# GinZhu/RDST

Measured on AMD Instinct MI355X. Metric: SR patches/sec fwd+bwd, RDST-E1 x4 64->256, higher is better.
Workload: dtype bf16; 1 GPU; RDST-E1 x4 (RDST_E1_OASIS_example_SRx4.ini), 1x64x64 LR patches -> 256x256, step = fwd + L1 + bwd + flat-bucket grad all-reduce + Adam; global_batch=32, per_gpu_batch=32, parallelism=dp1, hip_graph=True, grad_bucket_bytes=17859844

## Files before the change

rdst_amd/csrc/mlp3_mfma.hip:

```cpp
#include "linear.h"
#include "lds_dma.h"
#include "mfma.h"

#ifndef M3_ABL
#define M3_ABL 0
#endif

namespace {

constexpr int M3_TT = 128;


struct M3Args {
  const bf16* X; int64_t ldx; int x_bytes;
  const bf16* W1p; const float* sb1;
  const bf16* W2p; const float* sb2;
  bf16* Y; int64_t ldy;
  float* stats;
  int M, ntiles;
  unsigned long long* stamps;
};

#ifndef M3_NW90
#define M3_NW90 12
#endif
constexpr int m3_nw(int C) { return ((2 * C + 31) / 32) % 3 == 0 ? M3_NW90 : 8; }

template <int C>
struct M3Cfg {
  static constexpr int HID = 2 * C;
  static constexpr int KS1 = (C + 15) / 16, NT1 = (HID + 31) / 32;
  static constexpr int KS2 = (HID + 15) / 16, NT2 = (C + 31) / 32;
  static constexpr int XS = lds_kstep_stride(C), XSLOTS = XS / 16, XD = (2 * C + 15) / 16;
  static constexpr int TP = (M3_TT * XSLOTS + 63) / 64, TILEB = TP * 1024;
  static constexpr int HS = lds_kstep_stride(HID), HTILEB = M3_TT * HS;
  static constexpr int NW = m3_nw(C), NTHR = 64 * NW;
  static constexpr int NJ1 = (NT1 * 4 + NW - 1) / NW, P1 = NT1 / ce_gcd(NW, NT1), ND1 = NJ1 < P1 ? NJ1 : P1;
  static constexpr int NJ2 = (NT2 * 4 + NW - 1) / NW, P2 = NT2 / ce_gcd(NW, NT2), ND2 = NJ2 < P2 ? NJ2 : P2;
  static constexpr int NBUF = 2;
  static constexpr int CNT = (TP + NW - 1) / NW;
  static constexpr int H_OFF = NBUF * TILEB;
  static constexpr int STAT_OFF = H_OFF + HTILEB;
  static constexpr int SB1_OFF = STAT_OFF + NBUF * M3_TT * 2 * 4;
  static constexpr int SB1_B = (2 * NT1 * 32 * 4 + 1023) / 1024 * 1024;
  static constexpr int SB2_OFF = SB1_OFF + SB1_B;
  static constexpr int SB2_B = (2 * NT2 * 32 * 4 + 1023) / 1024 * 1024;
  static constexpr int TAB_OFF = SB2_OFF + SB2_B;
  static constexpr int SMEM = TAB_OFF + RDST_GELU_TAB4_BYTES;
  static constexpr int WGCU = SMEM <= 80 * 1024 ? 2 : 1;
  static_assert(SMEM <= 160 * 1024, "LDS");
  static_assert(TP >= NW, "every wave owns at least one piece of a tile");
  static_assert(CNT + 1 + 2 * ((NT2 * 4) / NW) < 64, "vmcnt is a 6-bit counter");
};

template <int C>
__global__ void __launch_bounds__(64 * m3_nw(C), M3Cfg<C>::WGCU == 2 ? (2 * m3_nw(C) + 3) / 4 : (m3_nw(C) + 3) / 4) mlp3_fwd_kernel(const M3Args p) {
  using CF = M3Cfg<C>;
  constexpr int KS1 = CF::KS1, KS2 = CF::KS2, NT1 = CF::NT1, NT2 = CF::NT2, XS = CF::XS, HS = CF::HS, NBUF = CF::NBUF, NW = CF::NW;
  constexpr int ND1 = CF::ND1, ND2 = CF::ND2, NJ1 = CF::NJ1, NJ2 = CF::NJ2, CNT = CF::CNT;
  extern __shared__ __attribute__((aligned(16))) char smem[];
  const int tid = threadIdx.x, lane = tid & 63, r = lane & 31, h = lane >> 5;
  const int wave = __builtin_amdgcn_readfirstlane(tid >> 6);
  float* statL = reinterpret_cast<float*>(smem + CF::STAT_OFF);
  const float* sb1L = reinterpret_cast<const float*>(smem + CF::SB1_OFF);
  const float* sb2L = reinterpret_cast<const float*>(smem + CF::SB2_OFF);
  char* hL = smem + CF::H_OFF;
  gelu_tab4_fill(smem + CF::TAB_OFF, tid, CF::NTHR);
  const char* gtab = smem + CF::TAB_OFF;

  const u32x4s_t rsx = dma_rsrc(p.X, (uint32_t)p.x_bytes), rs1 = dma_rsrc(p.sb1, 2 * NT1 * 32 * 4), rs2 = dma_rsrc(p.sb2, 2 * NT2 * 32 * 4);
  const uint32_t lds0 = lds_base(smem);
  const int grid = gridDim.x;
  RDST_PHASES_BEGIN(RDST_DBGV(p.stamps));
  u32x4v_t w1[ND1][KS1], w2[ND2][KS2];
#pragma unroll
  for (int jd = 0; jd < ND1; ++jd) {
    const int nt = (wave + NW * jd) % NT1;
#pragma unroll
    for (int ks = 0; ks < KS1; ++ks) {
      const char* src = reinterpret_cast<const char*>(p.W1p) + (((int64_t)nt * KS1 + ks) * 64 + lane) * 16;
      frag_load(w1[jd][ks], src);
    }
  }
#pragma unroll
  for (int jd = 0; jd < ND2; ++jd) {
    const int nt = (wave + NW * jd) % NT2;
#pragma unroll
    for (int ks = 0; ks < KS2; ++ks) {
      const char* src = reinterpret_cast<const char*>(p.W2p) + (((int64_t)nt * KS2 + ks) * 64 + lane) * 16;
      frag_load(w2[jd][ks], src);
    }
  }
  {
    constexpr int N1P = CF::SB1_B / 1024, N2P = CF::SB2_B / 1024;
    const int p1 = wave % N1P, p2 = wave % N2P;
    lds_dma16(rs1, __builtin_amdgcn_readfirstlane(lds0 + (uint32_t)(CF::SB1_OFF + p1 * 1024)), p1 * 1024 + lane * 16);
    lds_dma16(rs2, __builtin_amdgcn_readfirstlane(lds0 + (uint32_t)(CF::SB2_OFF + p2 * 1024)), p2 * 1024 + lane * 16);
  }
  auto issue_tile = [&](int tile, int b) {
#pragma unroll
    for (int i = 0; i < CNT; ++i) {
      int q = wave + NW * i;
      q = q < CF::TP ? q : q - NW;
      const int sidx = q * 64 + lane;
      const int tok = sidx / CF::XSLOTS, sl = sidx - tok * CF::XSLOTS;
      const int grow = tile * M3_TT + tok;
      const bool ok = tile < p.ntiles && tok < M3_TT && sl < CF::XD && grow < p.M;
      lds_dma16(rsx, __builtin_amdgcn_readfirstlane(lds0 + (uint32_t)(b * CF::TILEB + q * 1024)),
          ok ? grow * ((int)p.ldx * 2) + sl * 16 : p.x_bytes);
    }
  };
  static_assert(NBUF == 2, "the ring below is written for two buffers");
  issue_tile(blockIdx.x, 0);
  issue_tile(blockIdx.x + grid, 1);
  constexpr int NST = 1 + 2 * ((NT2 * 4) / NW);
  int kk = 0;
  for (int tile = blockIdx.x; tile < p.ntiles; tile += grid, ++kk) {
    const int b = kk & 1;
    if (kk == 0) wait_vmcnt<CNT>();
    else wait_vmcnt<CNT + NST>();
#pragma unroll
    for (int jd = 0; jd < ND1; ++jd)
#pragma unroll
      for (int ks = 0; ks < KS1; ++ks) frag_pin(w1[jd][ks]);
#pragma unroll
    for (int jd = 0; jd < ND2; ++jd)
#pragma unroll
      for (int ks = 0; ks < KS2; ++ks) frag_pin(w2[jd][ks]);
    __syncthreads();
    RDST_PHASE(RDST_DBGV(p.stamps), 0);
    const char* tb = smem + b * CF::TILEB;
    float* st = statL + b * M3_TT * 2;
    for (int tok = tid >> 2; tok < M3_TT; tok += CF::NTHR / 4) {
      const int part = tid & 3;
      constexpr int NSL = (CF::XD + 3) / 4;
      float xv[NSL][8];
      float sum = 0.f;
#pragma unroll
      for (int i = 0; i < NSL; ++i) {
        const int sl = part + 4 * i;
        const Pack16 q = *reinterpret_cast<const Pack16*>(tb + tok * XS + (sl < CF::XD ? sl : 0) * 16);
        Mma<bf16>::unpack(q, xv[i]);
#pragma unroll
        for (int e = 0; e < 8; ++e) {
          const bool valid = sl < CF::XD && sl * 8 + e < C;
          xv[i][e] = valid ? xv[i][e] : 0.f;
          sum += xv[i][e];
        }
      }
      sum += __shfl_xor(sum, 1, 64);
      sum += __shfl_xor(sum, 2, 64);
      const float mean = sum * (1.0f / C);
      float sq = 0.f;
#pragma unroll
      for (int i = 0; i < NSL; ++i) {
        const int sl = part + 4 * i;
#pragma unroll
        for (int e = 0; e < 8; ++e) {
          const bool valid = sl < CF::XD && sl * 8 + e < C;
          const float d = xv[i][e] - mean;
          sq = valid ? fmaf(d, d, sq) : sq;
        }
      }
      sq += __shfl_xor(sq, 1, 64);
      sq += __shfl_xor(sq, 2, 64);
      const float rstd = rsqrtf(sq * (1.0f / C) + 1e-5f);
      if (part == 0) {
        st[tok * 2] = mean;
        st[tok * 2 + 1] = rstd;
        const int grow = tile * M3_TT + tok;
        if (grow < p.M) *reinterpret_cast<float2*>(p.stats + (int64_t)grow * 2) = make_float2(mean, rstd);
      }
    }
    __syncthreads();
    RDST_PHASE(RDST_DBGV(p.stamps), 1);
#pragma unroll
    for (int jd = 0; jd < ND1; ++jd)
#pragma unroll 1
      for (int j = jd; j < NJ1; j += ND1) {
        const int item = wave + NW * j;
        if (item >= NT1 * 4) break;
        const int nt = item % NT1, tt = item / NT1;
        const int tok = tt * 32 + r;
        f32x16 acc;
#pragma unroll
        for (int v = 0; v < 16; ++v) acc[v] = 0.f;
        const char* brow = tb + tok * XS + h * 16;
#pragma unroll
        for (int ks = 0; ks < KS1; ++ks) {
          Pack16 bq = *reinterpret_cast<const Pack16*>(brow + ks * 32);
          if (C % 16 != 0 && ks == KS1 - 1) {
            constexpr int c0 = C % 16 < 8 ? C % 16 : 8, c1 = C % 16 > 8 ? C % 16 - 8 : 0;
#pragma unroll
            for (int d = 0; d < 4; ++d) bq.w[d] = (2 * d < (h ? c1 : c0)) ? bq.w[d] : 0u;
          }
          if (!(M3_ABL & 2)) acc = __builtin_amdgcn_mfma_f32_32x32x16_bf16(__builtin_bit_cast(bf16x8_t, w1[jd][ks]), __builtin_bit_cast(bf16x8_t, bq), acc, 0, 0, 0);
          else acc[ks & 15] += __uint_as_float(bq.w[0]);
        }
        const float2 mr = *reinterpret_cast<const float2*>(st + tok * 2);
        const float rstd = mr.y, nrm = -mr.y * mr.x;
        char* hrow = hL + tok * HS;
        float u[16], fr[16];
        uint32_t en[16];
#pragma unroll
        for (int g4 = 0; g4 < 4; ++g4) {
          const int n0 = nt * 32 + 8 * g4 + 4 * h;
          const float4 S4 = *reinterpret_cast<const float4*>(sb1L + n0);
          const float4 B4 = *reinterpret_cast<const float4*>(sb1L + NT1 * 32 + n0);
          u[4 * g4] = fmaf(rstd, acc[4 * g4], fmaf(nrm, S4.x, B4.x));
          u[4 * g4 + 1] = fmaf(rstd, acc[4 * g4 + 1], fmaf(nrm, S4.y, B4.y));
          u[4 * g4 + 2] = fmaf(rstd, acc[4 * g4 + 2], fmaf(nrm, S4.z, B4.z));
          u[4 * g4 + 3] = fmaf(rstd, acc[4 * g4 + 3], fmaf(nrm, S4.w, B4.w));
        }
#pragma unroll
        for (int v = 0; v < 16; ++v) {
          uint32_t off;
          if (M3_ABL & 1) { fr[v] = 0.f; en[v] = 0x3c003c00u; continue; }
          fr[v] = gelu_tab4_index(u[v], off);
          en[v] = *reinterpret_cast<const uint32_t*>(gtab + off);
        }
        __builtin_amdgcn_sched_barrier(0);
#pragma unroll
        for (int g4 = 0; g4 < 4; ++g4) {
          const int n0 = nt * 32 + 8 * g4 + 4 * h;
          const float h0 = u[4 * g4] * gelu_tab_lerp(fr[4 * g4], en[4 * g4]), h1 = u[4 * g4 + 1] * gelu_tab_lerp(fr[4 * g4 + 1], en[4 * g4 + 1]);
          const float h2 = u[4 * g4 + 2] * gelu_tab_lerp(fr[4 * g4 + 2], en[4 * g4 + 2]), h3 = u[4 * g4 + 3] * gelu_tab_lerp(fr[4 * g4 + 3], en[4 * g4 + 3]);
          u32x2_a4 uu;
          uu.x = pack_bf16x2(h0, h1); uu.y = pack_bf16x2(h2, h3);
          if (n0 * 2 + 8 <= HS) *reinterpret_cast<u32x2_a4*>(hrow + n0 * 2) = uu;
        }
      }
    RDST_PHASE(RDST_DBGV(p.stamps), 2);
    __syncthreads();
    RDST_PHASE(RDST_DBGV(p.stamps), 3);
#pragma unroll
    for (int jd = 0; jd < ND2; ++jd)
#pragma unroll 1
      for (int j = jd; j < NJ2; j += ND2) {
        const int item = wave + NW * j;
        if (item >= NT2 * 4) break;
        const int nt = item % NT2, tt = item / NT2;
        const int tok = tt * 32 + r;
        const int grow = tile * M3_TT + tok;
        f32x16 acc;
#pragma unroll
        for (int v = 0; v < 16; ++v) acc[v] = 0.f;
        const char* brow = hL + tok * HS + h * 16;
#pragma unroll
        for (int ks = 0; ks < KS2; ++ks) {
          const Pack16 bq = *reinterpret_cast<const Pack16*>(brow + ks * 32);
          if (!(M3_ABL & 4)) acc = __builtin_amdgcn_mfma_f32_32x32x16_bf16(__builtin_bit_cast(bf16x8_t, w2[jd][ks]), __builtin_bit_cast(bf16x8_t, bq), acc, 0, 0, 0);
          else acc[ks & 15] += __uint_as_float(bq.w[0]);
        }
#pragma unroll
        for (int g4 = 0; g4 < 4; ++g4) {
          const int n0 = nt * 32 + 8 * g4 + 4 * h;
          const float4 B4 = *reinterpret_cast<const float4*>(sb2L + NT2 * 32 + n0);
          uint32_t rx = 0u, ry = 0u;
          if (n0 < C) {
            const u32x2_a4 rr = *reinterpret_cast<const u32x2_a4*>(tb + tok * XS + n0 * 2);
            rx = rr.x; ry = rr.y;
          }
          acc[4 * g4] += B4.x + bf16lo(rx); acc[4 * g4 + 1] += B4.y + bf16hi(rx);
          acc[4 * g4 + 2] += B4.z + bf16lo(ry); acc[4 * g4 + 3] += B4.w + bf16hi(ry);
        }
        if (grow < p.M && !(M3_ABL & 8)) {
#pragma unroll
          for (int gp = 0; gp < 2; ++gp) {
            float c8[8];
#pragma unroll
            for (int e = 0; e < 4; ++e) {
              const auto sw = __builtin_amdgcn_permlane32_swap(__float_as_uint(acc[8 * gp + e]), __float_as_uint(acc[8 * gp + 4 + e]),
                                                               false, false);
              c8[e] = __uint_as_float(sw[0]);
              c8[4 + e] = __uint_as_float(sw[1]);
            }
            const int cb = nt * 32 + 8 * (2 * gp + h);
            const int nv = C - cb;
            if (nv <= 0) continue;
            bf16* yp = p.Y + (grow * (int)p.ldy + cb);
            if (nv >= 8) {
              u32x4_a4 u;
              u.x = pack_bf16x2(c8[0], c8[1]); u.y = pack_bf16x2(c8[2], c8[3]);
              u.z = pack_bf16x2(c8[4], c8[5]); u.w = pack_bf16x2(c8[6], c8[7]);
              *reinterpret_cast<u32x4_a4*>(yp) = u;
            } else {
#pragma unroll
              for (int d = 0; d < 3; ++d)
                if (2 * d + 2 <= nv) *reinterpret_cast<uint32_t*>(yp + 2 * d) = pack_bf16x2(c8[2 * d], c8[2 * d + 1]);
            }
          }
        }
      }
    RDST_PHASE(RDST_DBGV(p.stamps), 4);
    __syncthreads();
    issue_tile(tile + 2 * grid, b);
    RDST_PHASE(RDST_DBGV(p.stamps), 5);
  }
  RDST_PHASES_STORE(RDST_DBGV(p.stamps) && tid == 0, p.stamps, blockIdx.x);
}

template <int C>
int launch_m3(M3Args& p, hipStream_t st) {
  using CF = M3Cfg<C>;
  p.ntiles = (p.M + M3_TT - 1) / M3_TT;
  int grid = (p.ntiles + 1) / 2;
  if (grid > 256 * CF::WGCU) grid = 256 * CF::WGCU;
  if (grid < 1) grid = 1;
  auto kern = mlp3_fwd_kernel<C>;
  p.stamps = rdst_stamps_begin("RDST_M3_STAMPS", grid, 8, st);
  const int rc = rdst_launch(kern, dim3((unsigned)grid), dim3(CF::NTHR), CF::SMEM, st, "mlp3_fwd", p);
  rdst_stamps_end(p.stamps, grid, 8, RDST_STAMPS_SUMS, st, "mlp3_fwd: 0 wait+B0, 1 stats, 2 phase 1, 3 wait+B2, 4 phase 2, 5 B3+issue");
  return rc;
}

}

size_t mlp3_pack_bytes(int C, int hid) { return lin3_pack_bytes(C, hid) + lin3_pack_bytes(hid, C); }

bool mlp3_fwd_shape(int C, int hid) { return hid == 2 * C && (C == 60 || C == 90 || C == 120); }

int mlp3_fwd_bf16(const bf16* X, int64_t ldx, const float* ln_w, const float* ln_b, const float* W1, const float* b1, const float* W2,
                  const float* b2, bf16* Y, int64_t ldy, float* stats, int64_t M, int C, int hid, void* wpack, bool prepacked,
                  hipStream_t st) {
  if (!wpack || ((uintptr_t)wpack & 15) || !mlp3_fwd_shape(C, hid) || M <= 0) return RDST_ENOTSUP;
  if (((uintptr_t)X & 3) || (ldx & 1) || ((uintptr_t)Y & 3) || (ldy & 1)) return RDST_ENOTSUP;
  const int64_t xb = ((M - 1) * ldx + C) * 2;
  if (xb >= (1ll << 31) || M * ldy * 2 >= (1ll << 31)) return RDST_ENOTSUP;
  char* base = reinterpret_cast<char*>(wpack);
  char* base2 = base + lin3_pack_bytes(C, hid);
  if (!prepacked) {
    if (int rc = lin3_pack_launch(W1, ln_w, ln_b, b1, base, hid, C, 1.0f, st)) return rc;
    if (int rc = lin3_pack_launch(W2, nullptr, nullptr, b2, base2, C, hid, 1.0f, st)) return rc;
  }
  const int nt1 = (hid + 31) / 32, ks1 = (C + 15) / 16, nt2 = (C + 31) / 32, ks2 = (hid + 15) / 16;
  M3Args p{};
  p.X = X; p.ldx = ldx; p.x_bytes = (int)xb;
  p.W1p = reinterpret_cast<const bf16*>(base); p.sb1 = reinterpret_cast<const float*>(base + (size_t)nt1 * ks1 * 1024);
  p.W2p = reinterpret_cast<const bf16*>(base2); p.sb2 = reinterpret_cast<const float*>(base2 + (size_t)nt2 * ks2 * 1024);
  p.Y = Y; p.ldy = ldy; p.stats = stats; p.M = (int)M;
  if (C == 60) return launch_m3<60>(p, st);
  if (C == 90) return launch_m3<90>(p, st);
  return launch_m3<120>(p, st);
}
```

rdst_amd/csrc/mlp_mfma.hip:

```cpp
#include "linear.h"
#include "mfma.h"
#include "reduce_batch.h"
#include "wattn_hd.h"
#include <stdlib.h>

#ifdef MLP_ABL
#define MLP_DBG(p) (MLP_ABL)
#else
#define MLP_DBG(p) RDST_DBGV((p).dbg)
#endif

namespace {
using namespace wahd;
using MM = Mma<bf16>;

struct MlpArgs {
  const bf16* X; int64_t ldx; const float* stats; const float* lnw; const float* lnb;
  const float* W1; const float* b1; const float* W2; const float* b2;
  const bf16* dY; int64_t lddy; bf16* dX; int64_t lddx;
  float* slab; int64_t slab_stride;
  int64_t M; int C; int hid; int64_t ntiles; int tiles_per_wg;
  unsigned long long* stamps;
  int dbg;
};

template <int NCT> struct MlpCfg {
  static constexpr int NJ = 2 * NCT, NT = 64 * NJ, CP = 32 * NCT, JP = 32 * NJ;
  static constexpr int KC = CP / 16, KJ = JP / 16, PK = CP / 8;
  static constexpr int LDW = NCT == 4 ? 336 : CP * 2 + 16, LDX = LDW, LDH = 64;
  static constexpr int OFF_W1 = 0, OFF_XH = OFF_W1 + JP * LDW, OFF_DY = OFF_XH + 32 * LDX, OFF_DH = OFF_DY + 32 * LDX,
                       OFF_B1 = OFF_DH + JP * LDH, OFF_SM = OFF_B1 + JP * 4, OFF_RED = OFF_SM + 32 * 4,
                       OFF_TAB = OFF_RED + NCT * 32 * 8, OFF_W2L = OFF_TAB + RDST_GELU_TAB_BYTES;
  static constexpr int W2L = NCT == 4 ? 3 : 0, SMEM = OFF_W2L + W2L * NJ * 1024;
};

__device__ __forceinline__ void gelu_pair(f32x2 x, f32x2& cdf, f32x2& ex) {
  const f32x2 z = x * 0.70710678118654752440f;
  f32x2 az;
  az.x = __builtin_fabsf(z.x); az.y = __builtin_fabsf(z.y);
  const f32x2 den = __builtin_elementwise_fma(az, (f32x2)(0.3275911f), (f32x2)(1.0f));
  f32x2 t;
  t.x = __builtin_amdgcn_rcpf(den.x); t.y = __builtin_amdgcn_rcpf(den.y);
  f32x2 pl = __builtin_elementwise_fma(t, (f32x2)(0.5f * 1.061405429f), (f32x2)(0.5f * -1.453152027f));
  pl = __builtin_elementwise_fma(pl, t, (f32x2)(0.5f * 1.421413741f));
  pl = __builtin_elementwise_fma(pl, t, (f32x2)(0.5f * -0.284496736f));
  pl = __builtin_elementwise_fma(pl, t, (f32x2)(0.5f * 0.254829592f));
  pl = pl * t;
  const f32x2 a2 = (z * -1.4426950408889634f) * z;
  ex.x = __builtin_amdgcn_exp2f(a2.x); ex.y = __builtin_amdgcn_exp2f(a2.y);
  const f32x2 qn = pl * ex, qp = (f32x2)(1.0f) - qn;
  cdf.x = x.x >= 0.f ? qp.x : qn.x;
  cdf.y = x.y >= 0.f ? qp.y : qn.y;
}

template <int NCT, bool SPLIT>
__global__ void __launch_bounds__(128 * NCT, 2) mlp_bwd_kernel(const MlpArgs p) {
  using CF = MlpCfg<NCT>;
  extern __shared__ __attribute__((aligned(16))) char smem[];
  constexpr int NT = CF::NT, JP = CF::JP, LDW = CF::LDW, LDX = CF::LDX, PK = CF::PK, NJ = CF::NJ;
  const int tid = threadIdx.x, lane = tid & 63, wave = __builtin_amdgcn_readfirstlane(tid >> 6), r = lane & 31, hh = lane >> 5;
  const int C = p.C, hid = p.hid;
  const int j = 32 * wave + r;
  float* b1s = reinterpret_cast<float*>(smem + CF::OFF_B1);
  float* sm = reinterpret_cast<float*>(smem + CF::OFF_SM);
  float* red = reinterpret_cast<float*>(smem + CF::OFF_RED);
  const lds_cp gtab = (lds_cp)(smem + CF::OFF_TAB);
  gelu_tab_fill(smem + CF::OFF_TAB, tid, NT);
  int nst = 0;
  auto stamp = [&]() {
    if (RDST_DBGV(p.stamps) && tid == 0 && nst < 14) p.stamps[(size_t)blockIdx.x * 16 + nst++] = __builtin_readcyclecounter();
  };
  stamp();

  Pack16 w2b[CF::KC - CF::W2L];
  const lds_cp w2l = (lds_cp)(smem + CF::OFF_W2L + (wave * 64 + lane) * 16);
  {
    float f[CF::KC][8];
#pragma unroll
    for (int t = 0; t < CF::KC; ++t)
#pragma unroll
      for (int e = 0; e < 8; ++e) {
        const int c = 16 * t + 8 * hh + e;
        f[t][e] = p.W2[(int64_t)(c < C ? c : C - 1) * hid + (j < hid ? j : hid - 1)];
      }
#pragma unroll
    for (int t = 0; t < CF::KC; ++t) {
#pragma unroll
      for (int e = 0; e < 8; ++e) f[t][e] = (16 * t + 8 * hh + e < C && j < hid) ? f[t][e] : 0.f;
      if (t < CF::KC - CF::W2L) w2b[t < CF::KC - CF::W2L ? t : 0] = MM::pack(f[t]);
      else {
        const Pack16 pk = MM::pack(f[t]);
        u32x4_t v; v.x = pk.w[0]; v.y = pk.w[1]; v.z = pk.w[2]; v.w = pk.w[3];
        *reinterpret_cast<LDS_AS u32x4_t*>(w2l + (t - (CF::KC - CF::W2L)) * NJ * 1024) = v;
      }
    }
  }
  stamp();
  lds_zero16(smem + CF::OFF_W1, CF::OFF_DH - CF::OFF_W1, tid, NT);
  const int pk = tid % PK, jr = tid / PK, c0 = 8 * pk;
  {
    float gq[8], bq[8];
#pragma unroll
    for (int e = 0; e < 8; ++e) {
      const int c = c0 + e < C ? c0 + e : C - 1;
      gq[e] = p.lnw[c];
      bq[e] = p.lnb[c];
    }
#pragma unroll
    for (int e = 0; e < 8; ++e) {
      gq[e] = c0 + e < C ? gq[e] : 0.f;
      bq[e] = c0 + e < C ? bq[e] : 0.f;
    }
    const int cl = c0 < C - 8 ? c0 : C - 8, sh = c0 - cl;
    float w[NJ][8];
#pragma unroll
    for (int ps = 0; ps < NJ; ++ps) {
      const int jj = jr + 32 * ps;
      const float* src = p.W1 + (int64_t)(jj < hid ? jj : hid - 1) * C + cl;
      const u32x4_a4 a = *reinterpret_cast<const u32x4_a4*>(src), b = *reinterpret_cast<const u32x4_a4*>(src + 4);
      w[ps][0] = __uint_as_float(a.x); w[ps][1] = __uint_as_float(a.y); w[ps][2] = __uint_as_float(a.z); w[ps][3] = __uint_as_float(a.w);
      w[ps][4] = __uint_as_float(b.x); w[ps][5] = __uint_as_float(b.y); w[ps][6] = __uint_as_float(b.z); w[ps][7] = __uint_as_float(b.w);
    }
    if (sh != 0) {
#pragma unroll
      for (int ps = 0; ps < NJ; ++ps) {
        float t4[8], t2[8];
#pragma unroll
        for (int e = 0; e < 8; ++e) t4[e] = (sh & 4) ? (e + 4 < 8 ? w[ps][e + 4 < 8 ? e + 4 : 7] : 0.f) : w[ps][e];
#pragma unroll
        for (int e = 0; e < 8; ++e) t2[e] = (sh & 2) ? (e + 2 < 8 ? t4[e + 2 < 8 ? e + 2 : 7] : 0.f) : t4[e];
#pragma unroll
        for (int e = 0; e < 8; ++e) w[ps][e] = sh >= 8 ? 0.f : t2[e];
      }
    }
    __syncthreads();
    stamp();
    float* part = reinterpret_cast<float*>(smem + CF::OFF_DH);
#pragma unroll
    for (int ps = 0; ps < NJ; ++ps) {
      const int jj = jr + 32 * ps;
      if (jj < hid) {
        float f[8], dot = 0.f;
#pragma unroll
        for (int e = 0; e < 8; ++e) {
          f[e] = w[ps][e] * gq[e];
          dot = fmaf(w[ps][e], bq[e], dot);
        }
        *reinterpret_cast<Pack16*>(smem + CF::OFF_W1 + jj * LDW + c0 * 2) = MM::pack(f);
        part[jj * PK + pk] = dot;
      }
    }
    if (tid < 32) *reinterpret_cast<uint16_t*>(smem + CF::OFF_XH + tid * LDX + C * 2) = 0x3f80;
  }
  __syncthreads();
  stamp();
  {
    const float* part = reinterpret_cast<const float*>(smem + CF::OFF_DH);
    for (int jj = tid; jj < JP; jj += NT) {
      float v = 0.f;
      if (jj < hid) {
        v = p.b1 ? p.b1[jj] : 0.f;
#pragma unroll
        for (int k = 0; k < PK; ++k) v += part[jj * PK + k];
      }
      b1s[jj] = v;
    }
  }
  __syncthreads();

  stamp();
  constexpr int NU = SPLIT ? 2 : 1;
  const bool loader = SPLIT ? wave >= NCT : true;
  const int rowbytes = C * 2;
  int lrow[NU], loff[NU];
  bool lact[NU], lal[NU], lfirst[NU];
  const char* xp[NU];
  const char* yp[NU];
  const float* sp[NU];
#pragma unroll
  for (int u = 0; u < NU; ++u) {
    const int idx = SPLIT ? (tid - 64 * NCT) + 64 * NCT * u : tid;
    lrow[u] = (idx / PK) & 31;
    const int chk = idx - (idx / PK) * PK;
    lact[u] = loader && chk * 16 < rowbytes;
    int o = chk * 16;
    if (o + 16 > rowbytes) o = rowbytes - 16;
    if (!lact[u]) o = 0;
    loff[u] = o;
    lal[u] = (o & 15) == 0;
    lfirst[u] = lact[u] && chk == 0;
  }
  u32x4_a4 rx[NU], rdy[NU];
  float2 rst[NU];
  auto seek = [&](int64_t tile) {
#pragma unroll
    for (int u = 0; u < NU; ++u) {
      int64_t row = tile * 32 + lrow[u];
      row = row < p.M ? row : p.M - 1;
      xp[u] = reinterpret_cast<const char*>(p.X + row * p.ldx) + loff[u];
      yp[u] = reinterpret_cast<const char*>(p.dY + row * p.lddy) + loff[u];
      sp[u] = p.stats + 2 * row;
    }
  };
  auto fetch = [&]() {
#pragma unroll
    for (int u = 0; u < NU; ++u) {
      rx[u] = *reinterpret_cast<const u32x4_a4*>(xp[u]);
      rdy[u] = *reinterpret_cast<const u32x4_a4*>(yp[u]);
      rst[u] = *reinterpret_cast<const float2*>(sp[u]);
    }
  };
  const int64_t xstep = 32 * p.ldx * 2, ystep = 32 * p.lddy * 2;
  auto advance = [&]() {
#pragma unroll
    for (int u = 0; u < NU; ++u) {
      xp[u] += xstep;
      yp[u] += ystep;
      sp[u] += 64;
    }
  };
  auto put16 = [&](char* dst, const Pack16& v, bool aligned) {
    if (aligned) *reinterpret_cast<Pack16*>(dst) = v;
    else {
      uint32_t* d = reinterpret_cast<uint32_t*>(dst);
      d[0] = v.w[0]; d[1] = v.w[1]; d[2] = v.w[2]; d[3] = v.w[3];
    }
  };
  auto stash = [&](int64_t tile) {
#pragma unroll
    for (int u = 0; u < NU; ++u) {
      const bool valid = tile * 32 + lrow[u] < p.M;
      if (lact[u]) {
        float f[8];
        unpack8(rx[u], f);
#pragma unroll
        for (int e = 0; e < 8; ++e) f[e] = valid ? (f[e] - rst[u].x) * rst[u].y : 0.f;
        put16(smem + CF::OFF_XH + lrow[u] * LDX + loff[u], MM::pack(f), lal[u]);
        Pack16 d;
        d.w[0] = valid ? rdy[u].x : 0u; d.w[1] = valid ? rdy[u].y : 0u; d.w[2] = valid ? rdy[u].z : 0u; d.w[3] = valid ? rdy[u].w : 0u;
        put16(smem + CF::OFF_DY + lrow[u] * LDX + loff[u], d, lal[u]);
      }
    }
#pragma unroll
    for (int u = 0; u < NU; ++u)
      if (lfirst[u]) sm[lrow[u]] = rst[u].y;
  };

  const int q = (lane & 15) >> 2, pp = lane & 3, gq1 = (lane >> 4) & 1;
  const int sg = (r & 16) + 4 * (r & 3) + ((r >> 2) & 1) + 2 * ((r >> 3) & 1);
  const lds_cp xrow = (lds_cp)(smem + CF::OFF_XH + sg * LDX + hh * 16);
  const lds_cp yrow = (lds_cp)(smem + CF::OFF_DY + sg * LDX + hh * 16);
  const lds_cp wrow = (lds_cp)(smem + CF::OFF_W1 + j * LDW + hh * 16);
  const int dhpos = 32 * wave + (r & 16) + 4 * (r & 3) + ((r >> 2) & 3);
  const uint32_t dho = (uint32_t)dhpos * CF::LDH + 8u * ((dhpos >> 1) & 7);
  const lds_cp dhb = (lds_cp)(smem + CF::OFF_DH);
  const lds_cp xtr = (lds_cp)(smem + CF::OFF_XH + (4 * q + hh) * LDX + (16 * gq1 + 4 * pp) * 2);
  const lds_cp ytr = (lds_cp)(smem + CF::OFF_DY + (4 * q + hh) * LDX + (16 * gq1 + 4 * pp) * 2);
  const lds_cp wtr = (lds_cp)(smem + CF::OFF_W1 + (4 * q + hh) * LDW + (16 * gq1 + 4 * pp) * 2 + wave * 64);
  const lds_cp dtr0 = dhb + (4 * hh + q) * CF::LDH + 8 * ((4 * gq1 + pp) ^ ((2 * hh + (q >> 1)) & 7));
  const lds_cp dtr1 = dhb + (4 * hh + 8 + q) * CF::LDH + 8 * ((4 * gq1 + pp) ^ ((2 * hh + 4 + (q >> 1)) & 7));
  static_assert(CF::LDH == 64 && CF::OFF_DH % 64 == 0, "dHp image: 64-byte rows, XOR swizzle of the 8-byte pieces");

  f32x16 G1[NCT], W2g[NCT];
#pragma unroll
  for (int ct = 0; ct < NCT; ++ct)
#pragma unroll
    for (int v = 0; v < 16; ++v) { G1[ct][v] = 0.f; W2g[ct][v] = 0.f; }

  const int64_t t0 = (int64_t)blockIdx.x * p.tiles_per_wg;
  const int64_t t1 = t0 + p.tiles_per_wg < p.ntiles ? t0 + p.tiles_per_wg : p.ntiles;
  const float invC = 1.0f / (float)C;
  const int64_t full_tiles = p.M / 32;
  if (loader && t0 < t1) {
    seek(t0);
    fetch();
  }
  for (int64_t tile = t0; tile < t1; ++tile) {
    if (loader) {
      stash(tile);
      if (tile + 1 < t1) {
        if (tile + 1 < full_tiles) advance();
        else seek(tile + 1);
      }
      fetch();
    }
    __syncthreads();
    stamp();
    Pack16 hA[2], dA[2];
    {
      f32x16 ah, ad;
      const float bj = b1s[j];
#pragma unroll
      for (int v = 0; v < 16; ++v) { ah[v] = bj; ad[v] = 0.f; }
      if (!(MLP_DBG(p) & 2))
#pragma unroll
      for (int t = 0; t < CF::KC; ++t) {
        const Pack16 xa = lds_pack(xrow + 32 * t), wb = lds_pack(wrow + 32 * t), ya = lds_pack(yrow + 32 * t);
        MM::mma(ah, xa, wb);
        if (t < CF::KC - CF::W2L) MM::mma(ad, ya, w2b[t < CF::KC - CF::W2L ? t : 0]);
        else MM::mma(ad, ya, lds_pack(w2l + (t - (CF::KC - CF::W2L)) * NJ * 1024));
      }
      const bool ones = j == hid;
#pragma unroll
      for (int s = 0; s < 2; ++s) {
        constexpr int LB = NCT == 4 ? 4 : 8;
#pragma unroll
        for (int b = 0; b < 8; b += LB) {
          float fr[LB];
          u32x2_t en[LB];
#pragma unroll
          for (int k = 0; k < LB; ++k) {
            uint32_t off;
            fr[k] = gelu_tab_index(ah[8 * s + b + k], off);
            if (MLP_DBG(p) & 1) { en[k].x = off; en[k].y = off + 1; }
            else en[k] = *reinterpret_cast<const LDS_AS u32x2_t*>(gtab + off);
          }
          __builtin_amdgcn_sched_barrier(0);
#pragma unroll
          for (int k = 0; k < LB; k += 2) {
            const int v = 8 * s + b + k;
            const float h0 = ah[v] * gelu_tab_lerp(fr[k], en[k].x), h1 = ah[v + 1] * gelu_tab_lerp(fr[k + 1], en[k + 1].x);
            const float d0 = ad[v] * gelu_tab_lerp(fr[k], en[k].y), d1 = ad[v + 1] * gelu_tab_lerp(fr[k + 1], en[k + 1].y);
            const uint32_t hp = pack_bf16x2(h0, h1);
            hA[s].w[(b + k) / 2] = ones ? 0x3f803f80u : hp;
            dA[s].w[(b + k) / 2] = pack_bf16x2(d0, d1);
          }
        }
        u32x2_t lo, hi;
        lo.x = dA[s].w[0]; lo.y = dA[s].w[1]; hi.x = dA[s].w[2]; hi.y = dA[s].w[3];
        *reinterpret_cast<LDS_AS u32x2_t*>(dhb + (dho ^ (uint32_t)(8 * (4 * s + hh)))) = lo;
        *reinterpret_cast<LDS_AS u32x2_t*>(dhb + (dho ^ (uint32_t)(8 * (4 * s + 2 + hh)))) = hi;
      }
    }
    __syncthreads();
    stamp();
    if (!(MLP_DBG(p) & 4))
#pragma unroll
    for (int ct = 0; ct < NCT; ++ct)
#pragma unroll
      for (int s = 0; s < 2; ++s) {
        const Pack16 xb = lds_tr_pack(xtr + 16 * s * LDX + ct * 64, xtr + (16 * s + 2) * LDX + ct * 64);
        const Pack16 yb = lds_tr_pack(ytr + 16 * s * LDX + ct * 64, ytr + (16 * s + 2) * LDX + ct * 64);
        MM::mma(G1[ct], dA[s], xb);
        MM::mma(W2g[ct], hA[s], yb);
      }
    f32x16 dx;
    float rstd = 0.f;
    if (wave < NCT) {
      f32x16 dx2;
#pragma unroll
      for (int v = 0; v < 16; ++v) { dx[v] = 0.f; dx2[v] = 0.f; }
      if (!(MLP_DBG(p) & 8))
#pragma unroll
      for (int kk = 0; kk < CF::KJ; kk += 2) {
        const Pack16 wa = lds_tr_pack(wtr + 16 * kk * LDW, wtr + (16 * kk + 2) * LDW);
        const Pack16 db = lds_tr_pack(dtr0 + 16 * kk * CF::LDH, dtr1 + 16 * kk * CF::LDH);
        const Pack16 wa2 = lds_tr_pack(wtr + 16 * (kk + 1) * LDW, wtr + (16 * (kk + 1) + 2) * LDW);
        const Pack16 db2 = lds_tr_pack(dtr0 + 16 * (kk + 1) * CF::LDH, dtr1 + 16 * (kk + 1) * CF::LDH);
        MM::mma(dx, wa, db);
        MM::mma(dx2, wa2, db2);
      }
#pragma unroll
      for (int v = 0; v < 16; ++v) dx[v] += dx2[v];
      rstd = sm[sg];
      float s1 = 0.f, s2 = 0.f;
#pragma unroll
      for (int g4 = 0; g4 < 4; ++g4) {
        const u32x2_t xv = *reinterpret_cast<const LDS_AS u32x2_t*>((lds_cp)(smem + CF::OFF_XH + sg * LDX) + (32 * wave + 8 * g4 + 4 * hh) * 2);
        const float xh[4] = {bf16lo(xv.x), bf16hi(xv.x), bf16lo(xv.y), bf16hi(xv.y)};
#pragma unroll
        for (int e = 0; e < 4; ++e) {
          s1 += dx[4 * g4 + e];
          s2 = fmaf(dx[4 * g4 + e], xh[e], s2);
        }
      }
      s1 = half_swap_sum(s1);
      s2 = half_swap_sum(s2);
      if (hh == 0) *reinterpret_cast<float2*>(red + (wave * 32 + r) * 2) = make_float2(s1, s2);
    }
    __syncthreads();
    stamp();
    if (wave < NCT) {
      float s1 = 0.f, s2 = 0.f;
#pragma unroll
      for (int w = 0; w < NCT; ++w) {
        const float2 v = *reinterpret_cast<const float2*>(red + (w * 32 + r) * 2);
        s1 += v.x; s2 += v.y;
      }
      s1 *= invC; s2 *= invC;
      float o[16];
#pragma unroll
      for (int g4 = 0; g4 < 4; ++g4) {
        const int cb = (32 * wave + 8 * g4 + 4 * hh) * 2;
        const u32x2_t xv = *reinterpret_cast<const LDS_AS u32x2_t*>((lds_cp)(smem + CF::OFF_XH + sg * LDX) + cb);
        const u32x2_t yv = *reinterpret_cast<const LDS_AS u32x2_t*>((lds_cp)(smem + CF::OFF_DY + sg * LDX) + cb);
        const float xh[4] = {bf16lo(xv.x), bf16hi(xv.x), bf16lo(xv.y), bf16hi(xv.y)};
        const float dy[4] = {bf16lo(yv.x), bf16hi(yv.x), bf16lo(yv.y), bf16hi(yv.y)};
#pragma unroll
        for (int e = 0; e < 4; ++e) o[4 * g4 + e] = fmaf(rstd, dx[4 * g4 + e] - s1 - xh[e] * s2, dy[e]);
      }
      const int64_t row = tile * 32 + sg;
      if (row < p.M) {
        bf16* drow = p.dX + row * p.lddx;
#pragma unroll
        for (int gp = 0; gp < 2; ++gp) {
          float c8[8];
#pragma unroll
          for (int e = 0; e < 4; ++e) {
            const auto sw = __builtin_amdgcn_permlane32_swap(__float_as_uint(o[8 * gp + e]), __float_as_uint(o[8 * gp + 4 + e]), false, false);
            c8[e] = __uint_as_float(sw[0]);
            c8[4 + e] = __uint_as_float(sw[1]);
          }
          const int cb = 32 * wave + 8 * (2 * gp + hh);
          if (cb + 8 <= C) {
            u32x4_a4 u;
            u.x = pack_bf16x2(c8[0], c8[1]); u.y = pack_bf16x2(c8[2], c8[3]);
            u.z = pack_bf16x2(c8[4], c8[5]); u.w = pack_bf16x2(c8[6], c8[7]);
            *reinterpret_cast<u32x4_a4*>(drow + cb) = u;
          } else {
#pragma unroll
            for (int e = 0; e < 8; ++e)
              if (cb + e < C) drow[cb + e] = __float2bfloat16(c8[e]);
          }
        }
      }
    }
    __syncthreads();
    stamp();
  }
  if (RDST_DBGV(p.stamps) && tid == 0) p.stamps[(size_t)blockIdx.x * 16 + 14] = __builtin_readcyclecounter();
  uint2* my = reinterpret_cast<uint2*>(p.slab) + (int64_t)blockIdx.x * p.slab_stride;
  uint2* my2 = my + (int64_t)((hid + 3) / 4) * (C + 1);
#pragma unroll
  for (int ct = 0; ct < NCT; ++ct) {
    const int c = 32 * ct + r;
#pragma unroll
    for (int g4 = 0; g4 < 4; ++g4) {
      const int j0 = 32 * wave + 8 * g4 + 4 * hh;
      if (j0 < hid && c <= C)
        my[(int64_t)(j0 >> 2) * (C + 1) + c] = make_uint2(pack_bf16x2(G1[ct][4 * g4], G1[ct][4 * g4 + 1]), pack_bf16x2(G1[ct][4 * g4 + 2], G1[ct][4 * g4 + 3]));
      if (j0 <= hid && c < C)
        my2[(int64_t)(j0 >> 2) * C + c] = make_uint2(pack_bf16x2(W2g[ct][4 * g4], W2g[ct][4 * g4 + 1]), pack_bf16x2(W2g[ct][4 * g4 + 2], W2g[ct][4 * g4 + 3]));
    }
  }
  if (RDST_DBGV(p.stamps) && tid == 0) p.stamps[(size_t)blockIdx.x * 16 + 15] = __builtin_readcyclecounter();
}

template <int NCT> struct MlpFwdCfg {
  static constexpr int NJ = 2 * NCT, NT = 64 * NJ, CP = 32 * NCT, JP = 32 * NJ;
  static constexpr int KC = CP / 16, KJ = JP / 16, PK = CP / 8;
  static constexpr int LDW = CP * 2 + 16, LDX = CP * 2 + 16, LD2 = JP * 2 + 16;
  static constexpr int off_w2(int hid) { return hid * LDW; }
  static constexpr int off_x(int hid, int C) { return off_w2(hid) + C * LD2; }
  static constexpr int off_h(int hid, int C) { return off_x(hid, C) + 32 * LDX; }
  static constexpr int off_pst(int hid, int C) { return off_h(hid, C) + 32 * LD2; }
  static constexpr int off_s(int hid, int C) { return off_pst(hid, C) + 32 * 16 * 8; }
  static constexpr int smem(int hid, int C) { return off_s(hid, C) + 2 * JP * 4 + CP * 4; }
};

struct MlpFwdArgs {
  const bf16* X; int64_t ldx; const float* lnw; const float* lnb;
  const float* W1; const float* b1; const float* W2; const float* b2;
  bf16* Y; int64_t ldy; float* stats;
  int64_t M; int C; int hid; int64_t ntiles; int tiles_per_wg;
  unsigned long long* stamps;
};

template <int NCT>
__global__ void __launch_bounds__(128 * NCT, 2) mlp_fwd_kernel(const MlpFwdArgs p) {
  using CF = MlpFwdCfg<NCT>;
  extern __shared__ __attribute__((aligned(16))) char smem[];
  constexpr int NT = CF::NT, JP = CF::JP, CP = CF::CP, LDW = CF::LDW, LDX = CF::LDX, LD2 = CF::LD2, PK = CF::PK, NJ = CF::NJ;
  const int tid = threadIdx.x, lane = tid & 63, wave = __builtin_amdgcn_readfirstlane(tid >> 6), r = lane & 31, hh = lane >> 5;
  const int C = p.C, hid = p.hid;
  const int OFF_W2 = CF::off_w2(hid), OFF_X = CF::off_x(hid, C), OFF_H = CF::off_h(hid, C), OFF_PST = CF::off_pst(hid, C),
            OFF_S = CF::off_s(hid, C);
  float* Ss = reinterpret_cast<float*>(smem + OFF_S);
  float* b1s = Ss + JP;
  float* b2s = b1s + JP;
  float2* pst = reinterpret_cast<float2*>(smem + OFF_PST);
  int nst = 0;
  auto stamp = [&]() {
    if (RDST_DBGV(p.stamps) && tid == 0 && nst < 16) p.stamps[(size_t)blockIdx.x * 16 + nst++] = __builtin_readcyclecounter();
  };
  stamp();

  lds_zero16(smem, OFF_H, tid, NT);
  const int pk = tid % PK, jr = tid / PK, c0 = 8 * pk;
  {
    float gq[8], bq[8];
#pragma unroll
    for (int e = 0; e < 8; ++e) {
      const int c = c0 + e < C ? c0 + e : C - 1;
      gq[e] = p.lnw[c];
      bq[e] = p.lnb[c];
    }
#pragma unroll
    for (int e = 0; e < 8; ++e) {
      gq[e] = c0 + e < C ? gq[e] : 0.f;
      bq[e] = c0 + e < C ? bq[e] : 0.f;
    }
    const int cl = c0 < C - 8 ? c0 : C - 8, sh = c0 - cl;
    float w[NJ][8];
#pragma unroll
    for (int ps = 0; ps < NJ; ++ps) {
      const int jj = jr + 32 * ps;
      const float* src = p.W1 + (int64_t)(jj < hid ? jj : hid - 1) * C + cl;
      const u32x4_a4 a = *reinterpret_cast<const u32x4_a4*>(src), b = *reinterpret_cast<const u32x4_a4*>(src + 4);
      w[ps][0] = __uint_as_float(a.x); w[ps][1] = __uint_as_float(a.y); w[ps][2] = __uint_as_float(a.z); w[ps][3] = __uint_as_float(a.w);
      w[ps][4] = __uint_as_float(b.x); w[ps][5] = __uint_as_float(b.y); w[ps][6] = __uint_as_float(b.z); w[ps][7] = __uint_as_float(b.w);
    }
    if (sh != 0) {
#pragma unroll
      for (int ps = 0; ps < NJ; ++ps) {
        float t4[8], t2[8];
#pragma unroll
        for (int e = 0; e < 8; ++e) t4[e] = (sh & 4) ? (e + 4 < 8 ? w[ps][e + 4 < 8 ? e + 4 : 7] : 0.f) : w[ps][e];
#pragma unroll
        for (int e = 0; e < 8; ++e) t2[e] = (sh & 2) ? (e + 2 < 8 ? t4[e + 2 < 8 ? e + 2 : 7] : 0.f) : t4[e];
#pragma unroll
        for (int e = 0; e < 8; ++e) w[ps][e] = sh >= 8 ? 0.f : t2[e];
      }
    }
    __syncthreads();
    stamp();
    float* part = reinterpret_cast<float*>(smem + OFF_H);
#pragma unroll
    for (int ps = 0; ps < NJ; ++ps) {
      const int jj = jr + 32 * ps;
      if (jj < hid) {
        float f[8], dot = 0.f;
#pragma unroll
        for (int e = 0; e < 8; ++e) {
          f[e] = w[ps][e] * gq[e];
          dot = fmaf(w[ps][e], bq[e], dot);
        }
        *reinterpret_cast<Pack16*>(smem + jj * LDW + c0 * 2) = MM::pack(f);
        part[jj * PK + pk] = dot;
      }
    }
    stamp();
    const int P2 = (hid + 7) >> 3;
    for (int base = tid; base < C * P2; base += NT * 4) {
      float v[4][8];
#pragma unroll
      for (int u = 0; u < 4; ++u) {
        int idx = base + NT * u;
        idx = idx < C * P2 ? idx : C * P2 - 1;
        const int c = idx / P2, pq = idx - c * P2;
        const int k0 = 8 * pq < hid - 8 ? 8 * pq : hid - 8;
        const float* src = p.W2 + (int64_t)c * hid + k0;
        const u32x4_a4 a = *reinterpret_cast<const u32x4_a4*>(src), b = *reinterpret_cast<const u32x4_a4*>(src + 4);
        v[u][0] = __uint_as_float(a.x); v[u][1] = __uint_as_float(a.y); v[u][2] = __uint_as_float(a.z); v[u][3] = __uint_as_float(a.w);
        v[u][4] = __uint_as_float(b.x); v[u][5] = __uint_as_float(b.y); v[u][6] = __uint_as_float(b.z); v[u][7] = __uint_as_float(b.w);
      }
#pragma unroll
      for (int u = 0; u < 4; ++u) {
        const int idx = base + NT * u;
        if (idx < C * P2) {
          const int c = idx / P2, pq = idx - c * P2;
          const int k0 = 8 * pq < hid - 8 ? 8 * pq : hid - 8, s2 = 8 * pq - k0;
          float f[8];
#pragma unroll
          for (int e = 0; e < 8; ++e) {
            float x = 0.f;
#pragma unroll
            for (int k = 0; k < 8; ++k) x = (k == e + s2) ? v[u][k] : x;
            f[e] = x;
          }
          *reinterpret_cast<Pack16*>(smem + OFF_W2 + c * LD2 + pq * 16) = MM::pack(f);
        }
      }
    }
  }
  __syncthreads();
  stamp();
  {
    const float* part = reinterpret_cast<const float*>(smem + OFF_H);
    for (int jj = tid; jj < JP; jj += NT) {
      float v = 0.f, sv = 0.f;
      if (jj < hid) {
        v = p.b1 ? p.b1[jj] : 0.f;
#pragma unroll
        for (int k = 0; k < PK; ++k) {
          v += part[jj * PK + k];
          float fr[8];
          MM::unpack(*reinterpret_cast<const Pack16*>(smem + jj * LDW + k * 16), fr);
#pragma unroll
          for (int e = 0; e < 8; ++e) sv += fr[e];
        }
      }
      b1s[jj] = v;
// ... 344 lines not shown
```

Before: 1939 patches/s.

## Software-pipeline MLP3 forward MFMA with GELU/epilogue across token tiles

Adds an alternative schedule to the mlp3 forward kernel, enabled by default for C=90 and other non-60 widths. Each wave runs the next token tile's MFMA chain while it applies LayerNorm, GELU table lookup and bias+residual to the previous tile's accumulator, using double-buffered accumulators and sched barriers. The aim is to hide VALU and LDS epilogue latency behind matrix-core work. A similar interleave for the backward mlp kernel is added but stays off by default (MLP_SCHED=0). The trade-off is higher register pressure from the doubled accumulators and staged operands.

```diff
diff --git a/rdst_amd/csrc/mlp3_mfma.hip b/rdst_amd/csrc/mlp3_mfma.hip
--- a/rdst_amd/csrc/mlp3_mfma.hip
+++ b/rdst_amd/csrc/mlp3_mfma.hip
@@ -6,9 +6,14 @@
 #define M3_ABL 0
 #endif
 
+#ifndef M3_SCHED
+#define M3_SCHED 6
+#endif
+
 namespace {
 
 constexpr int M3_TT = 128;
+constexpr bool m3_sched(int C) { return (M3_SCHED & (C == 60 ? 1 : C == 90 ? 2 : 4)) != 0; }
 
 
 struct M3Args {
@@ -174,6 +179,88 @@
     }
     __syncthreads();
     RDST_PHASE(RDST_DBGV(p.stamps), 1);
+    if constexpr (m3_sched(C)) {
+      static_assert(ND1 == 1 && ND2 == 1 && NW % NT1 == 0 && NW % NT2 == 0 && (NT1 * 4) % NW == 0 && (NT2 * 4) % NW == 0,
+                    "one fragment set per wave and phase, and every wave owns the same number of items");
+      constexpr int NCH = 8;
+      {
+        const int nt = wave % NT1, tt0 = wave / NT1;
+        constexpr int TS = NW / NT1;
+        f32x16 acc[2];
+        Pack16 bq[KS1];
+#pragma unroll
+        for (int j = -1; j < NJ1; ++j) {
+          const bool cur = j >= 0, more = j + 1 < NJ1;
+          f32x16& an = acc[(j + 1) & 1];
+          const f32x16& ac = acc[j & 1];
+          const char* brow = tb + ((tt0 + TS * (more ? j + 1 : 0)) * 32 + r) * XS + h * 16;
+          auto load_b = [&](int ks) {
+            bq[ks] = *reinterpret_cast<const Pack16*>(brow + ks * 32);
+            if (C % 16 != 0 && ks == KS1 - 1) {
+              constexpr int c0 = C % 16 < 8 ? C % 16 : 8, c1 = C % 16 > 8 ? C % 16 - 8 : 0;
+#pragma unroll
+              for (int d = 0; d < 4; ++d) bq[ks].w[d] = (2 * d < (h ? c1 : c0)) ? bq[ks].w[d] : 0u;
+            }
+          };
+          if (more) {
+#pragma unroll
+            for (int ks = 0; ks < KS1; ++ks)
+              if (ks * NCH / KS1 == 0) load_b(ks);
+#pragma unroll
+            for (int v = 0; v < 16; ++v) an[v] = 0.f;
+          }
+          const int tok = (tt0 + TS * (cur ? j : 0)) * 32 + r;
+          float rstd = 0.f, nrm = 0.f;
+          if (cur) {
+            const float2 mr = *reinterpret_cast<const float2*>(st + tok * 2);
+            rstd = mr.y; nrm = -mr.y * mr.x;
+          }
+          char* hrow = hL + tok * HS;
+          float u[16], fr[16];
+          uint32_t en[16];
+          __builtin_amdgcn_sched_barrier(0);
+#pragma unroll
+          for (int ch = 0; ch < NCH; ++ch) {
+            if (more) {
+#pragma unroll
+              for (int ks = 0; ks < KS1; ++ks) {
+                if (ks * NCH / KS1 == ch + 1) load_b(ks);
+                if (ks * NCH / KS1 != ch) continue;
+                if (!(M3_ABL & 2)) an = __builtin_amdgcn_mfma_f32_32x32x16_bf16(__builtin_bit_cast(bf16x8_t, w1[0][ks]), __builtin_bit_cast(bf16x8_t, bq[ks]), an, 0, 0, 0);
+                else an[ks & 15] += __uint_as_float(bq[ks].w[0]);
+              }
+            }
+            const bool isA = (ch & 2) == 0;
+            const int g4 = (ch >> 2) * 2 + (ch & 1);
+            if (cur && isA) {
+              const int n0 = nt * 32 + 8 * g4 + 4 * h;
+              const float4 S4 = *reinterpret_cast<const float4*>(sb1L + n0);
+              const float4 B4 = *reinterpret_cast<const float4*>(sb1L + NT1 * 32 + n0);
+              u[4 * g4] = fmaf(rstd, ac[4 * g4], fmaf(nrm, S4.x, B4.x));
+              u[4 * g4 + 1] = fmaf(rstd, ac[4 * g4 + 1], fmaf(nrm, S4.y, B4.y));
+              u[4 * g4 + 2] = fmaf(rstd, ac[4 * g4 + 2], fmaf(nrm, S4.z, B4.z));
+              u[4 * g4 + 3] = fmaf(rstd, ac[4 * g4 + 3], fmaf(nrm, S4.w, B4.w));
+#pragma unroll
+              for (int v = 4 * g4; v < 4 * g4 + 4; ++v) {
+                uint32_t off;
+                if (M3_ABL & 1) { fr[v] = 0.f; en[v] = 0x3c003c00u; continue; }
+                fr[v] = gelu_tab4_index(u[v], off);
+                en[v] = *reinterpret_cast<const uint32_t*>(gtab + off);
+              }
+            }
+            if (cur && !isA) {
+              const int n0 = nt * 32 + 8 * g4 + 4 * h;
+              const float h0 = u[4 * g4] * gelu_tab_lerp(fr[4 * g4], en[4 * g4]), h1 = u[4 * g4 + 1] * gelu_tab_lerp(fr[4 * g4 + 1], en[4 * g4 + 1]);
+              const float h2 = u[4 * g4 + 2] * gelu_tab_lerp(fr[4 * g4 + 2], en[4 * g4 + 2]), h3 = u[4 * g4 + 3] * gelu_tab_lerp(fr[4 * g4 + 3], en[4 * g4 + 3]);
+              u32x2_a4 uu;
+              uu.x = pack_bf16x2(h0, h1); uu.y = pack_bf16x2(h2, h3);
+              if (n0 * 2 + 8 <= HS) *reinterpret_cast<u32x2_a4*>(hrow + n0 * 2) = uu;
+            }
+            __builtin_amdgcn_sched_barrier(0);
+          }
+        }
+      }
+    } else {
 #pragma unroll
     for (int jd = 0; jd < ND1; ++jd)
 #pragma unroll 1
@@ -230,9 +317,90 @@
           if (n0 * 2 + 8 <= HS) *reinterpret_cast<u32x2_a4*>(hrow + n0 * 2) = uu;
         }
       }
+    }
     RDST_PHASE(RDST_DBGV(p.stamps), 2);
     __syncthreads();
     RDST_PHASE(RDST_DBGV(p.stamps), 3);
+    if constexpr (m3_sched(C) && NJ2 > 1) {
+      static_assert(ND2 == 1 && NW % NT2 == 0 && (NT2 * 4) % NW == 0, "one fragment set per wave, the same number of items in every wave");
+      constexpr int NCH = 8;
+      {
+        const int nt = wave % NT2, tt0 = wave / NT2;
+        constexpr int TS = NW / NT2;
+        f32x16 acc[2];
+        float bx[2][16];
+        Pack16 bq[KS2];
+#pragma unroll
+        for (int j = -1; j < NJ2; ++j) {
+          const bool cur = j >= 0, more = j + 1 < NJ2;
+          f32x16& an = acc[(j + 1) & 1];
+          f32x16& ac = acc[j & 1];
+          const int tok = (tt0 + TS * (cur ? j : 0)) * 32 + r, tokn = (tt0 + TS * (more ? j + 1 : 0)) * 32 + r;
+          const int grow = tile * M3_TT + tok;
+          const char* brow = hL + tokn * HS + h * 16;
+          if (more) {
+#pragma unroll
+            for (int v = 0; v < 16; ++v) an[v] = 0.f;
+#pragma unroll
+            for (int ks = 0; ks < KS2; ++ks)
+              if (ks * NCH / KS2 == 0) bq[ks] = *reinterpret_cast<const Pack16*>(brow + ks * 32);
+          }
+          __builtin_amdgcn_sched_barrier(0);
+#pragma unroll
+          for (int ch = 0; ch < NCH; ++ch) {
+            if (more) {
+#pragma unroll
+              for (int ks = 0; ks < KS2; ++ks) {
+                if (ks * NCH / KS2 == ch + 1) bq[ks] = *reinterpret_cast<const Pack16*>(brow + ks * 32);
+                if (ks * NCH / KS2 != ch) continue;
+                if (!(M3_ABL & 4)) an = __builtin_amdgcn_mfma_f32_32x32x16_bf16(__builtin_bit_cast(bf16x8_t, w2[0][ks]), __builtin_bit_cast(bf16x8_t, bq[ks]), an, 0, 0, 0);
+                else an[ks & 15] += __uint_as_float(bq[ks].w[0]);
+              }
+            }
+            if (cur && ch < 2) {
+#pragma unroll
+              for (int v = 8 * ch; v < 8 * ch + 8; ++v) ac[v] += bx[j & 1][v];
+            }
+            if (cur && (ch == 2 || ch == 3)) {
+              const int gp = ch - 2;
+              float c8[8];
+#pragma unroll
+              for (int e = 0; e < 4; ++e) {
+                const auto sw = __builtin_amdgcn_permlane32_swap(__float_as_uint(ac[8 * gp + e]), __float_as_uint(ac[8 * gp + 4 + e]),
+                                                                 false, false);
+                c8[e] = __uint_as_float(sw[0]);
+                c8[4 + e] = __uint_as_float(sw[1]);
+              }
+              const int cb = nt * 32 + 8 * (2 * gp + h);
+              const int nv = C - cb;
+              bf16* yp = p.Y + (grow * (int)p.ldy + cb);
+              u32x4_a4 uo;
+              uo.x = pack_bf16x2(c8[0], c8[1]); uo.y = pack_bf16x2(c8[2], c8[3]);
+              uo.z = pack_bf16x2(c8[4], c8[5]); uo.w = pack_bf16x2(c8[6], c8[7]);
+              if (grow < p.M && !(M3_ABL & 8)) {
+                if (nv >= 8) *reinterpret_cast<u32x4_a4*>(yp) = uo;
+                else {
+                  const uint32_t ud[3] = {uo.x, uo.y, uo.z};
+#pragma unroll
+                  for (int d = 0; d < 3; ++d)
+                    if (2 * d + 2 <= nv) *reinterpret_cast<uint32_t*>(yp + 2 * d) = ud[d];
+                }
+              }
+            }
+            if (more && ch >= 4) {
+              const int g4 = ch - 4, n0 = nt * 32 + 8 * g4 + 4 * h;
+              const float4 B4 = *reinterpret_cast<const float4*>(sb2L + NT2 * 32 + n0);
+              const u32x2_a4 rr = *reinterpret_cast<const u32x2_a4*>(tb + tokn * XS + (n0 < C ? n0 : 0) * 2);
+              const uint32_t rx = n0 < C ? rr.x : 0u, ry = n0 < C ? rr.y : 0u;
+              float* b4 = bx[(j + 1) & 1] + 4 * g4;
+              b4[0] = B4.x + bf16lo(rx); b4[1] = B4.y + bf16hi(rx);
+              b4[2] = B4.z + bf16lo(ry); b4[3] = B4.w + bf16hi(ry);
+            }
+            __builtin_amdgcn_sched_barrier(0);
+          }
+        }
+      }
+    } else {
 #pragma unroll
     for (int jd = 0; jd < ND2; ++jd)
 #pragma unroll 1
@@ -292,6 +460,7 @@
           }
         }
       }
+    }
     RDST_PHASE(RDST_DBGV(p.stamps), 4);
     __syncthreads();
     issue_tile(tile + 2 * grid, b);
diff --git a/rdst_amd/csrc/mlp_mfma.hip b/rdst_amd/csrc/mlp_mfma.hip
--- a/rdst_amd/csrc/mlp_mfma.hip
+++ b/rdst_amd/csrc/mlp_mfma.hip
@@ -10,10 +10,14 @@
 #define MLP_DBG(p) RDST_DBGV((p).dbg)
 #endif
 
+#ifndef MLP_SCHED
+#define MLP_SCHED 0
+#endif
+
 namespace {
 using namespace wahd;
 using MM = Mma<bf16>;
-
+constexpr bool mlp_sched(int NCT) { return (MLP_SCHED & (NCT == 2 ? 1 : NCT == 3 ? 2 : 4)) != 0; }
 struct MlpArgs {
   const bf16* X; int64_t ldx; const float* stats; const float* lnw; const float* lnb;
   const float* W1; const float* b1; const float* W2; const float* b2;
@@ -287,7 +291,56 @@
     __syncthreads();
     stamp();
     Pack16 hA[2], dA[2];
-    {
+    if constexpr (mlp_sched(NCT) && !SPLIT) {
+      f32x16 ah, ad;
+      const float bj = b1s[j];
+#pragma unroll
+      for (int v = 0; v < 16; ++v) { ah[v] = bj; ad[v] = 0.f; }
+      if (!(MLP_DBG(p) & 2))
+#pragma unroll
+      for (int t = 0; t < CF::KC; ++t) MM::mma(ah, lds_pack(xrow + 32 * t), lds_pack(wrow + 32 * t));
+      const bool ones = j == hid;
+      float fr[16];
+      u32x2_t en[16];
+      auto h_pair = [&](int P) {
+        const float h0 = ah[2 * P] * gelu_tab_lerp(fr[2 * P], en[2 * P].x), h1 = ah[2 * P + 1] * gelu_tab_lerp(fr[2 * P + 1], en[2 * P + 1].x);
+        hA[P / 4].w[P % 4] = ones ? 0x3f803f80u : pack_bf16x2(h0, h1);
+      };
+      __builtin_amdgcn_sched_barrier(0);
+#pragma unroll
+      for (int t = 0; t < CF::KC; ++t) {
+        if (!(MLP_DBG(p) & 2)) {
+          const Pack16 ya = lds_pack(yrow + 32 * t);
+          if (t < CF::KC - CF::W2L) MM::mma(ad, ya, w2b[t < CF::KC - CF::W2L ? t : 0]);
+          else MM::mma(ad, ya, lds_pack(w2l + (t - (CF::KC - CF::W2L)) * NJ * 1024));
+        }
+#pragma unroll
+        for (int v = 2 * (8 * t / CF::KC); v < 2 * (8 * (t + 1) / CF::KC); ++v) {
+          uint32_t off;
+          fr[v] = gelu_tab_index(ah[v], off);
+          if (MLP_DBG(p) & 1) { en[v].x = off; en[v].y = off + 1; }
+          else en[v] = *reinterpret_cast<const LDS_AS u32x2_t*>(gtab + off);
+        }
+        if (t > 0)
+#pragma unroll
+          for (int P = 8 * (t - 1) / CF::KC; P < 8 * t / CF::KC; ++P) h_pair(P);
+        __builtin_amdgcn_sched_barrier(0);
+      }
+#pragma unroll
+      for (int P = 8 * (CF::KC - 1) / CF::KC; P < 8; ++P) h_pair(P);
+#pragma unroll
+      for (int s = 0; s < 2; ++s) {
+#pragma unroll
+        for (int P = 4 * s; P < 4 * s + 4; ++P) {
+          const float d0 = ad[2 * P] * gelu_tab_lerp(fr[2 * P], en[2 * P].y), d1 = ad[2 * P + 1] * gelu_tab_lerp(fr[2 * P + 1], en[2 * P + 1].y);
+          dA[s].w[P % 4] = pack_bf16x2(d0, d1);
+        }
+        u32x2_t lo, hi;
+        lo.x = dA[s].w[0]; lo.y = dA[s].w[1]; hi.x = dA[s].w[2]; hi.y = dA[s].w[3];
+        *reinterpret_cast<LDS_AS u32x2_t*>(dhb + (dho ^ (uint32_t)(8 * (4 * s + hh)))) = lo;
+        *reinterpret_cast<LDS_AS u32x2_t*>(dhb + (dho ^ (uint32_t)(8 * (4 * s + 2 + hh)))) = hi;
+      }
+    } else {
       f32x16 ah, ad;
       const float bj = b1s[j];
 #pragma unroll
```

Result: no change. 1936 patches/s (median of 3 runs) (-0.2%).
